# ICLDisco/ompi

Measured on AMD Instinct MI355X. Metric: Allreduce busBW GB/s @256MiB fp32 SUM at 2/4/8 GPUs; MPI_Op HBM GB/s, higher is better.
Workload: dtype f32; 1 GPU; MPI_Op 3-buffer SUM fp32, 1 GiB per buffer (BASELINE configs[1]); count=268435456, bytes_per_buffer=1073741824, op=MPI_SUM, datatype=MPI_FLOAT, kernel=op_vec_kernel<float,SUM,3buff>

## Files before the change

ompi_amd/csrc/coll_ipc.hip:

```cpp
#include <hip/hip_runtime.h>

#include <sched.h>
#include <unistd.h>

#include <algorithm>
#include <array>
#include <atomic>
#include <chrono>
#include <cstdarg>
#include <cstdio>
#include <cstdlib>
#include <cstring>
#include <deque>
#include <map>
#include <memory>
#include <mutex>
#include <new>
#include <utility>
#include <vector>

#include "../../include/ompi_amd_coll.h"
#include "bootstrap.h"
#include "comm_internal.h"
#include "host_mark.h"
// ... 1232 lines not shown
    if (want > kMaxIpcBytes) {
        record_msg("landing buffer of %zu bytes exceeds the %zu-byte IPC mapping limit", want,
                   kMaxIpcBytes);
        return OMPI_AMD_ERR_UNSUPPORTED;
    }
    land_blob mine{};
    char *fresh = nullptr;
    const hipError_t e = alloc_exportable(want, &fresh, &mine.d.h);
    mine.token = landing_token(c->rank);
    if (e == hipSuccess) land_desc(fresh, want, &mine.d);
    else record_hip(e, "landing buffer (deferred growth): hipMalloc / hipIpcGetMemHandle");
    mine.ok = e == hipSuccess;
    pending_op g{};
    g.kind = PEND_GROW;
    g.stream = s;
    g.grow = fresh;
    g.grow_bytes = want;
    g.grow_token = mine.token;
    const int rc = nb_ticket(c, g, &mine, sizeof(mine));
    if (rc != OMPI_AMD_SUCCESS) {
        release_exportable(fresh);
        return rc;
    }
    c->pending.push_back(g);
    c->npending.fetch_add(1);
    c->land_planned = want - kLandTag;
    return OMPI_AMD_SUCCESS;
}

static int launch_barrier(ompi_amd_comm_t *c, hipStream_t s);

static int grow_launch(ompi_amd_comm_t *c, const pending_op &g, const land_blob *all) {
    const size_t want = g.grow_bytes;
    ipc_ref *refs[kMaxRanks] = {};
    void *maps[kMaxRanks] = {};
    int status = all[c->rank].ok ? 0 : 1;
    for (int p = 0; p < c->size && status == 0; ++p) {
        if (p == c->rank) continue;
        if (!all[p].ok) {
            record_msg("landing buffer: rank %d failed to allocate or export its buffer", p);
            status = 1;
        } else if (ipc_map(alloc_of(all[p].d), c, &refs[p], &maps[p]) != OMPI_AMD_SUCCESS) {
            status = 1;
        }
    }
    if (status == 0) {
        tok_ptrs peers{};
        tok_set expect{};
        for (int p = 0; p < c->size; ++p) {
            expect.t[p] = all[p].token;
            if (p != c->rank) peers.p[p] = (const uint64_t *)((char *)maps[p] + want - kLandTag);
        }
        note_stream(c, g.stream);
        hipLaunchKernelGGL(land_stamp_kernel, dim3(1), dim3(1), 0, g.stream,
                           (uint64_t *)(g.grow + want - kLandTag), g.grow_token);
        int rc = record_hip(hipGetLastError(), "landing stamp launch (deferred growth)");
        if (rc == OMPI_AMD_SUCCESS) rc = launch_barrier(c, g.stream);
        if (rc == OMPI_AMD_SUCCESS) {
            hipLaunchKernelGGL(land_check_kernel, dim3(1), dim3(64), 0, g.stream, peers, expect, c->rank,
                               c->size, c->err_dev, c->flags + kAbortWord);
            rc = record_hip(hipGetLastError(), "landing check launch (deferred growth)");
        }
        if (rc != OMPI_AMD_SUCCESS) status = 1;
    }
    for (int q = 0; q < c->size; ++q) c->land_tokens.push_back(all[q].token);
    if (status != 0) {
        for (int p = 0; p < kMaxRanks; ++p) ipc_unmap(refs[p], c);
        if (g.grow) c->land_retired.push_back(g.grow);
        c->land_failed = true;
        return OMPI_AMD_ERR_HIP;
    }
    if (c->land) c->land_retired.push_back(c->land);
    for (int p = 0; p < kMaxRanks; ++p) {
        if (c->land_ref[p]) c->land_ref_retired.push_back(c->land_ref[p]);
        c->land_ref[p] = refs[p];
    }
    c->land = g.grow;
    for (int p = 0; p < c->size; ++p)
        c->peer_land.p[p] = p == c->rank ? c->land : (const char *)ipc_ref_base(c->land_ref[p]);
    c->land_bytes = want - kLandTag;
    ++c->deferred_growths;
    return OMPI_AMD_SUCCESS;
}

static int launch_barrier(ompi_amd_comm_t *c, hipStream_t s) {
    note_stream(c, s);
    ++c->epoch;
    const uint64_t ticks = (uint64_t)c->timeout_ms * 100000ull;
    hipLaunchKernelGGL(barrier_kernel, dim3(1), dim3(64), 0, s, c->flags, c->peer_flags, c->rank,
                       c->size, c->epoch, c->err_dev, ticks, c->dbg_dev);
    return record_hip(hipGetLastError(), "barrier launch");
}

static int launch_copy(ompi_amd_comm_t *c, const cp_jobs &jobs, hipStream_t s) {
    if (jobs.n == 0) return OMPI_AMD_SUCCESS;
    note_stream(c, s);
    int64_t most = 0;
    for (int i = 0; i < jobs.n; ++i) most = std::max(most, jobs.j[i].bytes);
    int64_t blocks = (most / 16 + kXferThreads * 4 - 1) / (kXferThreads * 4);
    blocks = std::max<int64_t>(1, std::min<int64_t>(blocks, std::max(1, c->max_blocks / jobs.n)));
    if (c->copy_nt)
        hipLaunchKernelGGL(copy_kernel<true>, dim3((unsigned)blocks, (unsigned)jobs.n),
                           dim3(kXferThreads), 0, s, jobs);
    else
        hipLaunchKernelGGL(copy_kernel<false>, dim3((unsigned)blocks, (unsigned)jobs.n),
                           dim3(kXferThreads), 0, s, jobs);
    return record_hip(hipGetLastError(), "copy launch");
}


static int arena_alloc(ompi_amd_comm_t *c, size_t need, char **out,
                       size_t min_chunk = (size_t)64 << 20) {
    host_step st("arena_alloc", need);
    const size_t n = (std::max<size_t>(need, 1) + 255) & ~(size_t)255;
    std::lock_guard<std::mutex> g(c->arena_mu);
    for (auto &ch : c->arena) {
        for (auto it = ch.free.begin(); it != ch.free.end(); ++it) {
            if (it->second < n) continue;
            const size_t off = it->first, left = it->second - n;
            ch.free.erase(it);
            if (left) ch.free[off + n] = left;
            ch.used[off] = n;
            *out = ch.base + off;
            return OMPI_AMD_SUCCESS;
        }
    }
    if (n > kMaxIpcBytes) {
        record_msg("shadow of %zu bytes exceeds the %zu-byte IPC allocation limit", n, kMaxIpcBytes);
        return OMPI_AMD_ERR_UNSUPPORTED;
    }
    const size_t want = std::min(kMaxIpcBytes,
                                 (std::max({n, min_chunk, c->arena_bytes}) + (2u << 20) - 1) &
                                     ~(size_t)((2u << 20) - 1));
    char *mem = nullptr;
    hipIpcMemHandle_t h;
    const hipError_t e = alloc_exportable(want, &mem, &h);
    if (e != hipSuccess) return record_hip(e, "shadow arena: hipMalloc / hipIpcGetMemHandle");
    c->arena.push_back({mem, want, {}, {}});
    auto &ch = c->arena.back();
    if (want > n) ch.free[n] = want - n;
    ch.used[0] = n;
    c->arena_bytes += want;
    *out = mem;
    return OMPI_AMD_SUCCESS;
}

static void arena_free(ompi_amd_comm_t *c, char *p) {
    if (!p) return;
    std::lock_guard<std::mutex> g(c->arena_mu);
    for (auto &ch : c->arena) {
        if (p < ch.base || p >= ch.base + ch.size) continue;
        const size_t off = (size_t)(p - ch.base);
        auto u = ch.used.find(off);
        if (u == ch.used.end()) return;
        size_t lo = off, len = u->second;
        ch.used.erase(u);
        auto nx = ch.free.lower_bound(off);
        if (nx != ch.free.end() && nx->first == off + len) {
            len += nx->second;
            nx = ch.free.erase(nx);
        }
        if (nx != ch.free.begin()) {
            auto pv = std::prev(nx);
            if (pv->first + pv->second == lo) {
                lo = pv->first;
                len += pv->second;
                ch.free.erase(pv);
            }
        }
        ch.free[lo] = len;
        return;
    }
}

static int shadow_reserve(ompi_amd_comm_t *c, size_t need, char **out, int k = 0) {
    char *&sh = k ? c->shadow2 : c->shadow;
    size_t &bytes = k ? c->shadow2_bytes : c->shadow_bytes;
    if (need <= bytes) {
        *out = sh;
        return OMPI_AMD_SUCCESS;
    }
    TRY(quiesce(c, "quiesce (shadow growth)"));
    arena_free(c, sh);
    const size_t want = std::max(need, std::min(2 * bytes, kMaxIpcBytes));
    sh = nullptr;
    bytes = 0;
    TRY(arena_alloc(c, want, &sh));
    bytes = want;
    *out = sh;
    return OMPI_AMD_SUCCESS;
}

static int shadow_plan(ompi_amd_comm_t *c, const void **src, size_t sbytes, void **rbuf,
                       size_t rbytes, bool rbuf_in, bool owned, shadow_set *post,
                       bool split_inplace = false) {
    *post = shadow_set{};
    bool inplace = *src && *src == (const void *)*rbuf;
    bool fs = false, fr = false;
    buf_desc d;
    if (*src && sbytes) {
        if (c->force_shadow || !c->user_ipc) {
            fs = true;
        } else {
            const int rc = export_buf(c, *src, &d, &fs);
            if (rc != OMPI_AMD_SUCCESS && !fs) return rc;
        }
    }
    if (inplace && fs && split_inplace) {
        inplace = false;
        fr = true;
        rbuf_in = false;
    } else if (inplace) {
        fr = fs;
        fs = false;
        rbytes = std::max(rbytes, sbytes);
        rbuf_in = true;
    } else if (*rbuf && rbytes) {
        if (c->force_shadow || !c->user_ipc) {
            fr = true;
        } else {
            const int rc = export_buf(c, *rbuf, &d, &fr);
            if (rc != OMPI_AMD_SUCCESS && !fr) return rc;
        }
    }
    if (!fs && !fr) return OMPI_AMD_SUCCESS;
    const size_t so = fs ? ((uintptr_t)*src & 255) : 0;
    const size_t rbase = fs ? ((so + sbytes + 255) & ~(size_t)255) : 0;
    const size_t ro = fr ? rbase + ((uintptr_t)*rbuf & 255) : rbase;
    size_t need = (fr ? ro + rbytes : so + sbytes) + 256;
    const bool split2 = fs && fr && need > kMaxIpcBytes;
    if (split2) need = so + sbytes + 256;
    char *mem = nullptr, *mem2 = nullptr;
    if (owned) {
        TRY(arena_alloc(c, need, &mem));
        post->mem = mem;
        if (split2) {
            TRY(arena_alloc(c, ((uintptr_t)*rbuf & 255) + rbytes + 256, &mem2));
            post->mem2 = mem2;
        }
    } else {
        TRY(shadow_reserve(c, need, &mem));
        if (split2) TRY(shadow_reserve(c, ((uintptr_t)*rbuf & 255) + rbytes + 256, &mem2, 1));
    }
    if (fs) {
        post->in.j[post->in.n++] = {(const char *)*src, mem + so, (int64_t)sbytes};
        *src = mem + so;
    }
    if (fr) {
        char *r = split2 ? mem2 + ((uintptr_t)*rbuf & 255) : mem + ro;
        if (rbuf_in) post->in.j[post->in.n++] = {(const char *)*rbuf, r, (int64_t)rbytes};
        post->out = {r, (char *)*rbuf, (int64_t)rbytes};
        *rbuf = r;
        if (inplace) *src = r;
    }
    ++c->shadowed;
    return OMPI_AMD_SUCCESS;
}

static int shadow_in(ompi_amd_comm_t *c, const shadow_set &sh, hipStream_t s) {
    return launch_copy(c, sh.in, s);
}

static int shadow_out(ompi_amd_comm_t *c, const shadow_set &sh, hipStream_t s) {
    if (sh.out.bytes <= 0) return OMPI_AMD_SUCCESS;
    cp_jobs cj{};
    cj.j[0] = sh.out;
    cj.n = 1;
    return launch_copy(c, cj, s);
}

static ptr_set one_ptr(const void *p) {
    ptr_set r{};
    r.p[0] = (const char *)p;
    return r;
}

static ptr_set push_order(const ompi_amd_comm_t *c, const ptr_set &bufs) {
    ptr_set r{};
    for (int k = 0; k < c->size; ++k) r.p[k] = bufs.p[(c->rank + k) % c->size];
    return r;
}

static int launch_reduce_core(int op, int type, const ptr_set &src, int nsrc, const ptr_set &dst,
                              int ndst, int order, int flags, red_jobs jobs, int max_blocks,
                              bool nt_store, hipStream_t s) {
    red_launch_fn f = red_fn(op, type);
    if (!f) return OMPI_AMD_ERR_UNSUPPORTED;
    if (jobs.n == 0 || nsrc < 1) return OMPI_AMD_SUCCESS;
    const size_t ext = ompi_amd_type_extent(type);
    int64_t most = 0;
    for (int i = 0; i < jobs.n; ++i) {
        red_job &j = jobs.j[i];
        const uintptr_t ph = (uintptr_t)(dst.p[0] + j.off_dst * ext) & 15;
        bool same = ext <= 16 && 16 % ext == 0;
        for (int r = 0; r < nsrc; ++r)
            same = same && ((((uintptr_t)(src.p[r] + j.off * ext)) & 15) == ph);
        for (int d = 1; d < ndst; ++d)
            same = same && ((((uintptr_t)(dst.p[d] + j.off_dst * ext)) & 15) == ph);
        const int64_t lead = (int64_t)((16 - ph) & 15);
        j.head = (same && lead % (int64_t)ext == 0) ? (int)std::min<int64_t>(lead / (int64_t)ext, j.cnt) : -1;
        most = std::max(most, j.cnt);
    }
    if (most == 0) return OMPI_AMD_SUCCESS;
    const int64_t per = (int64_t)(16 / ext) * kXferThreads;
    int64_t blocks = (most + per - 1) / per;
    blocks = std::max<int64_t>(1, std::min<int64_t>(blocks, std::max(1, max_blocks / jobs.n)));
    return record_hip(f(dim3((unsigned)blocks, (unsigned)jobs.n), src, dst, ndst, nsrc, order,
                        flags | (nt_store ? FOLD_NT_STORE : 0), jobs, s),
                      "reduce launch");
}

static int launch_reduce(ompi_amd_comm_t *c, int op, int type, const ptr_set &src, int nsrc,
                         const ptr_set &dst, int ndst, int order, int flags, const red_jobs &jobs,
                         hipStream_t s) {
    if (!red_fn(op, type)) return OMPI_AMD_ERR_UNSUPPORTED;
    if (jobs.n == 0 || nsrc < 1) return OMPI_AMD_SUCCESS;
    note_stream(c, s);
    return launch_reduce_core(op, type, src, nsrc, dst, ndst, order, flags, jobs, c->max_blocks,
                              c->copy_nt != 0, s);
}

static hipEvent_t prof_event(ompi_amd_comm_t *c) {
    if (!c->ev_free.empty()) {
        hipEvent_t e = c->ev_free.back();
        c->ev_free.pop_back();
        return e;
    }
    hipEvent_t e = nullptr;
    if (hipEventCreate(&e) != hipSuccess) return nullptr;
    return e;
}

template <typename F>
static int timed_phase(ompi_amd_comm_t *c, int phase, hipStream_t s, F &&launch) {
    if (!c->profile) return launch();
    hipEvent_t a = prof_event(c), b = prof_event(c);
    if (a) hip_ignore(hipEventRecord(a, s));
    const int rc = launch();
    if (b) hip_ignore(hipEventRecord(b, s));
    if (a && b) c->ev_phase[phase].emplace_back(a, b);
    return rc;
}

static int check_sticky(ompi_amd_comm_t *c) {
    const int e = __atomic_load_n(c->err_host, __ATOMIC_ACQUIRE);
    if (e != 0) {
        record_msg("collective device error %d (a peer did not reach a barrier within %lld ms)",
                   e, (long long)c->timeout_ms);
        return e;
    }
    return OMPI_AMD_SUCCESS;
}

static bool in_place(const void *sbuf, const void *rbuf) {
    return sbuf == rbuf || sbuf == (const void *)1;
}

struct stage_half {
    char *mine;
    ptr_set peers;
};
static stage_half next_half(ompi_amd_comm_t *c) {
    const size_t h = (size_t)(c->stage_seq++ & 1) * c->scratch_bytes;
    stage_half r;
    r.mine = c->scratch + h;
    for (int p = 0; p < kMaxRanks; ++p) r.peers.p[p] = c->peer_scratch.p[p] ? c->peer_scratch.p[p] + h : nullptr;
    return r;
}

static void ring_jobs(int64_t count, int n, red_jobs *jobs, int only_block) {
    int64_t split, early, late;
    blockcount(count, n, &split, &early, &late);
    jobs->n = 0;
    for (int b = 0; b < n; ++b) {
        if (only_block >= 0 && b != only_block) continue;
        red_job &j = jobs->j[jobs->n++];
        j.off = block_off(b, split, early, late);
        j.cnt = block_cnt(b, split, early, late);
        j.off_dst = j.off;
        j.first = b;
        j.head = -1;
    }
}

static int pof2_floor(int n) {
    int a = 1;
    while (a * 2 <= n) a *= 2;
    return a;
}

static fold_plan allreduce_fold(int n, int tuned_alg, size_t count, int type, bool root0_inplace,
                                int red_alg = 0) {
    const size_t msg = type_size(type) * count;
    const fold_plan tree{ORDER_TREE, 0, 0}, ring{ORDER_RING, 0, 0};
    const fold_plan linear{ORDER_CHAIN, 0, 0};
    switch (tuned_alg) {
    case TUNED_AR_BASIC_LINEAR: return linear;
    case TUNED_AR_NONOVERLAPPING: {
        const red_order ro = tuned_reduce_order(n, msg, count, 0, root0_inplace, red_alg);
        return {ro.order, ro.first, ro.flags};
    }
    case TUNED_AR_RECURSIVE_DOUBLING: return tree;
    case TUNED_AR_RING:
    case TUNED_AR_RING_SEGMENTED:
        return count < (size_t)n ? tree : ring;
    case TUNED_AR_RABENSEIFNER:
        return count < (size_t)pof2_floor(n) ? linear : fold_plan{ORDER_RABEN, 0, 0};
    default:
        return (msg < 10000 || count < (size_t)n) ? tree : ring;
    }
}

static void raben_piece(int64_t count, int n, int o, int64_t *lo, int64_t *cnt) {
    int64_t l = 0, w = count;
    for (int m = 1; m < pof2_floor(n); m <<= 1) {
        const int64_t half = w / 2;
        if (o & m) { l += half; w -= half; }
        else w = half;
    }
    *lo = l;
    *cnt = w;
}

static void fold_jobs(const fold_plan &p, int64_t count, int n, int block, red_jobs *jobs) {
    if (p.order == ORDER_RING) {
        ring_jobs(count, n, jobs, block);
        return;
    }
    int64_t lo = 0, hi = count;
    if (block >= 0) {
        int64_t split, early, late;
        blockcount(count, n, &split, &early, &late);
        lo = block_off(block, split, early, late);
        hi = lo + block_cnt(block, split, early, late);
    }
    jobs->n = 0;
    if (p.order != ORDER_RABEN) {
        red_job &j = jobs->j[jobs->n++];
        j = red_job{lo, hi - lo, lo, p.first, -1};
        return;
    }
    const int adj = pof2_floor(n);
    for (int o = 0; o < adj; ++o) {
        int64_t plo, pcnt;
        raben_piece(count, n, o, &plo, &pcnt);
        const int64_t a = std::max(lo, plo), b = std::min(hi, plo + pcnt);
        if (a >= b) continue;
        red_job &j = jobs->j[jobs->n++];
        j = red_job{a, b - a, a, 0, -1};
        j.aux = o << 8;
    }
}

static red_jobs one_job(int64_t off, int64_t cnt, int64_t off_dst, int first) {
    red_jobs jobs;
    jobs.n = 1;
    jobs.j[0] = {off, cnt, off_dst, first, -1};
    return jobs;
}
static int scan_sources(int rank, bool exclusive) { return exclusive ? rank : rank + 1; }

static int stage_in(ompi_amd_comm_t *c, const void *src, size_t bytes, stage_half *sh,
                    hipStream_t s) {
    if (bytes > c->scratch_bytes) {
        record_msg("staged collective of %zu B exceeds the %zu B scratch", bytes, c->scratch_bytes);
        return OMPI_AMD_ERR_BAD_PARAM;
    }
    *sh = next_half(c);
    cp_jobs cj{};
    cj.n = 1;
    cj.j[0] = {(const char *)src, sh->mine, (int64_t)bytes};
    TRY(launch_copy(c, cj, s));
    return launch_barrier(c, s);
}

static int allreduce_fused(ompi_amd_comm_t *c, const void *src, void *rbuf, int64_t count,
                           int op, int type, bool tree, hipStream_t s) {
    fused_launch_fn f = fused_fn(op, type);
    if (!f) return OMPI_AMD_ERR_UNSUPPORTED;
    note_stream(c, s);
    const int n = c->size;
    const stage_half sh = next_half(c);
    fused_args a{};
    a.src = (const char *)src;
    a.dst = (char *)rbuf;
    a.mine = sh.mine;
    a.peers = sh.peers;
    a.flags = c->flags;
    a.peer_flags = c->peer_flags;
    a.rank = c->rank;
    a.n = n;
    a.order = tree ? ORDER_TREE : ORDER_RING;
    a.count = count;
    blockcount(count, n, &a.split, &a.early, &a.late);
    a.epoch = ++c->epoch;
    a.timeout_ticks = (uint64_t)c->timeout_ms * 100000ull;
    a.err = c->err_dev;
    const int rows = tree ? 1 : n;
    const int64_t most = tree ? count : a.early;
    const int64_t cols = std::max<int64_t>(
        1, std::min<int64_t>((most + 4 * kXferThreads - 1) / (4 * kXferThreads),
                             kFusedMaxGroups / rows));
    if (c->want_mark && c->mark_word) {
        a.done = reinterpret_cast<uint32_t *>(c->flags) + kFusedDoneWord + kFusedDoneStride * c->mark_slot;
        a.mark = c->mark_word;
        a.mark_v = mark_reserve();
    }
    TRY(record_hip(f(dim3((unsigned)cols, (unsigned)rows), a, s), "fused allreduce launch"));
    if (a.mark) c->mark_embedded = a.mark_v;
    return OMPI_AMD_SUCCESS;
}

static size_t two_shot_result_off(size_t bytes) { return (bytes + 255) & ~(size_t)255; }

static bool two_shot_fits(const ompi_amd_comm_t *c, int64_t count, size_t ext) {
    int64_t split, early, late;
    blockcount(count, c->size, &split, &early, &late);
    return two_shot_result_off((size_t)count * ext) + (size_t)early * ext + 16 <= c->scratch_bytes;
}

static int allreduce_staged_two_shot(ompi_amd_comm_t *c, const void *src, void *rbuf,
                                     int64_t count, int op, int type, const fold_plan &fp,
                                     hipStream_t s) {
    const int n = c->size, mine = (c->rank + 1) % n;
    const int64_t ext = (int64_t)ompi_amd_type_extent(type);
    const size_t res = two_shot_result_off((size_t)count * ext);
    int64_t split, early, late;
    blockcount(count, n, &split, &early, &late);
    stage_half sh;
    TRY(stage_in(c, src, (size_t)(count * ext), &sh, s));
    const int64_t offm = block_off(mine, split, early, late) * ext;
    ptr_set dst{};
    dst.p[0] = (const char *)rbuf;
    dst.p[1] = sh.mine + res + (offm & 15) - offm;
    red_jobs jobs;
    fold_jobs(fp, count, n, mine, &jobs);
    TRY(launch_reduce(c, op, type, sh.peers, n, dst, 2, fp.order, fp.flags, jobs, s));
    TRY(launch_barrier(c, s));
    cp_jobs cj{};
    for (int b = 0; b < n; ++b) {
        if (b == mine) continue;
        const int owner = (b + n - 1) % n;
        const int64_t off = block_off(b, split, early, late) * ext;
        cj.j[cj.n++] = {sh.peers.p[owner] + res + (off & 15), (char *)rbuf + off,
                        block_cnt(b, split, early, late) * ext};
    }
    return launch_copy(c, cj, s);
}

static int allreduce_pull(ompi_amd_comm_t *c, const ptr_set &sp, const ptr_set &rp, void *rbuf,
                          int64_t count, int op, int type, const fold_plan &fp, hipStream_t s) {
    const int n = c->size, mine = (c->rank + 1) % n;
    const int64_t ext = (int64_t)ompi_amd_type_extent(type);
    TRY(launch_barrier(c, s));
    red_jobs jobs;
    fold_jobs(fp, count, n, mine, &jobs);
    TRY(timed_phase(c, 0, s, [&] {
        return launch_reduce(c, op, type, sp, n, one_ptr(rbuf), 1, fp.order, fp.flags, jobs, s);
    }));
    TRY(launch_barrier(c, s));
    int64_t split, early, late;
    blockcount(count, n, &split, &early, &late);
    cp_jobs cj{};
    for (int b = 0; b < n; ++b) {
        if (b == mine) continue;
        const int owner = (b + n - 1) % n;
        const int64_t off = block_off(b, split, early, late) * ext;
        cj.j[cj.n++] = {rp.p[owner] + off, (char *)rbuf + off, block_cnt(b, split, early, late) * ext};
    }
    TRY(timed_phase(c, 1, s, [&] { return launch_copy(c, cj, s); }));
    return launch_barrier(c, s);
}

static int allreduce_pull_staged(ompi_amd_comm_t *c, const ptr_set &sp, char *sh, void *rbuf,
                                 int64_t count, int op, int type, const fold_plan &fp,
                                 hipStream_t s) {
    const int n = c->size, mine = (c->rank + 1) % n;
    const int64_t ext = (int64_t)ompi_amd_type_extent(type);
    TRY(launch_barrier(c, s));
    red_jobs jobs;
    fold_jobs(fp, count, n, mine, &jobs);
    ptr_set dsts{};
    dsts.p[0] = (const char *)rbuf;
    dsts.p[1] = sh;
    TRY(timed_phase(c, 0, s, [&] {
        return launch_reduce(c, op, type, sp, n, dsts, 2, fp.order, fp.flags, jobs, s);
    }));
    TRY(launch_barrier(c, s));
    int64_t split, early, late;
    blockcount(count, n, &split, &early, &late);
    cp_jobs cj{};
    for (int b = 0; b < n; ++b) {
        if (b == mine) continue;
        const int owner = (b + n - 1) % n;
        const int64_t off = block_off(b, split, early, late) * ext;
        cj.j[cj.n++] = {sp.p[owner] + off, (char *)rbuf + off, block_cnt(b, split, early, late) * ext};
    }
    TRY(timed_phase(c, 1, s, [&] { return launch_copy(c, cj, s); }));
    return launch_barrier(c, s);
}

static int allreduce_pull_push(ompi_amd_comm_t *c, const ptr_set &sp, const ptr_set &rp,
                               int64_t count, int op, int type, const fold_plan &fp,
                               hipStream_t s) {
    const int n = c->size, mine = (c->rank + 1) % n;
    TRY(launch_barrier(c, s));
    red_jobs jobs;
    fold_jobs(fp, count, n, mine, &jobs);
    const ptr_set dsts = push_order(c, rp);
// ... 3026 lines not shown
```

ompi_amd/csrc/coll_kern.hip:

```cpp
#include <hip/hip_runtime.h>

#include <algorithm>
#include <array>
#include <utility>

#include "coll_kernels.h"

#ifndef COLL_OP
#error "build with -DCOLL_OP=<op index>"
#endif

namespace ompi_amd {
namespace {

template <int OP, int TYPE>
hipError_t red_launch_slot(dim3 grid, const ptr_set &src, const ptr_set &dst, int ndst, int n,
                           int order, int flags, const red_jobs &jobs, hipStream_t s) {
    if constexpr (slot_supported(OP, TYPE)) {
        using T = typename type_of<TYPE>::type;
        if (n <= 8)
            hipLaunchKernelGGL((reduce_kernel<T, OP, 8>), grid, dim3(kXferThreads), 0, s, src, dst,
                               ndst, n, order, flags, jobs);
        else
            hipLaunchKernelGGL((reduce_kernel<T, OP, kMaxRanks>), grid, dim3(kXferThreads), 0, s,
                               src, dst, ndst, n, order, flags, jobs);
        return hipGetLastError();
    } else {
        return hipErrorInvalidValue;
    }
}

template <int OP, int TYPE>
hipError_t fused_launch_slot(dim3 grid, const fused_args &a, hipStream_t s) {
    if constexpr (slot_supported(OP, TYPE)) {
        using T = typename type_of<TYPE>::type;
        hipLaunchKernelGGL((fused_allreduce_kernel<T, OP>), grid, dim3(kXferThreads), 0, s, a);
        return hipGetLastError();
    } else {
        return hipErrorInvalidValue;
    }
}

template <int OP, int TYPE>
hipError_t pipe_launch_slot(unsigned groups, const pipe_args &a, hipStream_t s) {
    if constexpr (slot_supported(OP, TYPE)) {
        using T = typename type_of<TYPE>::type;
        if (a.n > 8) return hipErrorInvalidValue;
        static const int64_t cap = [] {
            int per_cu = 0, cus = 0, dev = 0;
            if (hipGetDevice(&dev) != hipSuccess ||
                hipOccupancyMaxActiveBlocksPerMultiprocessor(
                    &per_cu, reinterpret_cast<const void *>(&pipe_allreduce_kernel<T, OP, 8>),
                    kXferThreads, 0) != hipSuccess ||
                hipDeviceGetAttribute(&cus, hipDeviceAttributeMultiprocessorCount, dev) != hipSuccess) {
                (void)hipGetLastError();
                return (int64_t)64;
            }
            return std::max<int64_t>(1, (int64_t)per_cu * cus / 2);
        }();
        const int64_t fit = std::max<int64_t>(1, cap / std::max(1, a.colocated));
        const dim3 g((unsigned)std::min<int64_t>(groups, fit)), b(kXferThreads);
        hipLaunchKernelGGL((pipe_allreduce_kernel<T, OP, 8>), g, b, 0, s, a);
        return hipGetLastError();
    } else {
        return hipErrorInvalidValue;
    }
}

template <int OP, int... T>
constexpr std::array<red_launch_fn, OMPI_AMD_TYPE_COUNT> make_red_row(std::integer_sequence<int, T...>) {
    return {{(slot_supported(OP, T) ? &red_launch_slot<OP, T> : (red_launch_fn) nullptr)...}};
}
template <int OP, int... T>
constexpr std::array<fused_launch_fn, OMPI_AMD_TYPE_COUNT> make_fused_row(
    std::integer_sequence<int, T...>) {
    return {{(slot_supported(OP, T) ? &fused_launch_slot<OP, T> : (fused_launch_fn) nullptr)...}};
}

template <int OP, int... T>
constexpr std::array<pipe_launch_fn, OMPI_AMD_TYPE_COUNT> make_pipe_row(
    std::integer_sequence<int, T...>) {
    return {{(slot_supported(OP, T) ? &pipe_launch_slot<OP, T> : (pipe_launch_fn) nullptr)...}};
}

const auto g_red_row = make_red_row<COLL_OP>(std::make_integer_sequence<int, OMPI_AMD_TYPE_COUNT>{});
const auto g_fused_row = make_fused_row<COLL_OP>(std::make_integer_sequence<int, OMPI_AMD_TYPE_COUNT>{});
const auto g_pipe_row = make_pipe_row<COLL_OP>(std::make_integer_sequence<int, OMPI_AMD_TYPE_COUNT>{});

}

#define ROW_NAME2(a, b) a##b
#define ROW_NAME(a, b) ROW_NAME2(a, b)
const red_launch_fn *ROW_NAME(red_row_, COLL_OP)() { return g_red_row.data(); }
const fused_launch_fn *ROW_NAME(fused_row_, COLL_OP)() { return g_fused_row.data(); }
const pipe_launch_fn *ROW_NAME(pipe_row_, COLL_OP)() { return g_pipe_row.data(); }

}
```

ompi_amd/csrc/coll_kernels.h:

```cpp
#pragma once

#include <hip/hip_runtime.h>

#include <cstdint>

#include "../../include/ompi_amd_coll.h"
#include "op_device.h"

namespace ompi_amd {

constexpr int kMaxRanks = OMPI_AMD_MAX_RANKS;
constexpr int kXferThreads = 256;

struct ptr_set { const char *p[kMaxRanks]; };
struct flag_set { uint64_t *p[kMaxRanks]; };

enum order_t {
    ORDER_RING = 0,
    ORDER_TREE = 1,
    ORDER_CHAIN = 2,
    ORDER_BINOMIAL = 3,
    ORDER_BINARY = 4,
    ORDER_HALVING = 5,
    ORDER_RABEN = 6,
};
constexpr int FOLD_ROOT_INPLACE = 1;
constexpr int FOLD_NT_STORE = 1 << 16;

struct red_job {
    int64_t off, cnt, off_dst;
    int first;
    int head;
    int aux = 0;
};
struct red_jobs { red_job j[2 * kMaxRanks]; int n; };

struct cp_job { const char *src; char *dst; int64_t bytes; };
struct cp_jobs { cp_job j[kMaxRanks]; int n; };

__device__ __forceinline__ void sys_acquire() {
    __builtin_amdgcn_fence(__ATOMIC_ACQUIRE, "");
    asm volatile("s_waitcnt vmcnt(0)" ::: "memory");
}
__device__ __forceinline__ void sys_release() {
    __builtin_amdgcn_fence(__ATOMIC_RELEASE, "");
    asm volatile("s_waitcnt vmcnt(0)" ::: "memory");
}

__device__ __forceinline__ void acquire_once() {
    if (threadIdx.x == 0) sys_acquire();
    __syncthreads();
}

constexpr int kAbortWord = 512;
constexpr size_t kFlagPageBytes = 8192;

__device__ __forceinline__ bool wait_epoch(const uint64_t *flag, uint64_t epoch, int *err,
                                           uint64_t ticks, uint64_t *abort_word,
                                           uint64_t *seen = nullptr) {
    const uint64_t t0 = __builtin_amdgcn_s_memrealtime();
    uint64_t check = t0 + 100000;
    while (__hip_atomic_load(flag, __ATOMIC_RELAXED, __HIP_MEMORY_SCOPE_SYSTEM) < epoch) {
        __builtin_amdgcn_s_sleep(1);
        const uint64_t now = __builtin_amdgcn_s_memrealtime();
        if (now - t0 > ticks) {
            __hip_atomic_store(err, (int)OMPI_AMD_ERR_TIMEOUT, __ATOMIC_RELAXED,
                               __HIP_MEMORY_SCOPE_SYSTEM);
            __hip_atomic_store(abort_word, (uint64_t)1, __ATOMIC_RELAXED, __HIP_MEMORY_SCOPE_SYSTEM);
            return false;
        }
        if (now >= check) {
            if (seen)
                __hip_atomic_store(seen, __hip_atomic_load(flag, __ATOMIC_RELAXED, __HIP_MEMORY_SCOPE_SYSTEM),
                                   __ATOMIC_RELAXED, __HIP_MEMORY_SCOPE_SYSTEM);
            if (__hip_atomic_load(abort_word, __ATOMIC_RELAXED, __HIP_MEMORY_SCOPE_SYSTEM) != 0) {
                __hip_atomic_store(err, (int)OMPI_AMD_ERR_TIMEOUT, __ATOMIC_RELAXED,
                                   __HIP_MEMORY_SCOPE_SYSTEM);
                return false;
            }
            check = now + 100000;
        }
    }
    return true;
}

__device__ __forceinline__ void xfer_epilogue() {
    asm volatile("s_waitcnt vmcnt(0)" ::: "memory");
    __syncthreads();
    if (threadIdx.x == 0) sys_release();
}

template <typename T, int OP, int NM = kMaxRanks>
__device__ __forceinline__ T fold(const T (&v)[NM], int n, int order, int flags) {
    using F = opfn<OP, false>;
    const bool swap = (flags & FOLD_ROOT_INPLACE) != 0;
    if (order == ORDER_RING) {
        T acc = v[0];
#pragma unroll
        for (int j = 1; j < NM; ++j)
            if (j < n) acc = F::template f<T>(v[j], acc);
        return acc;
    }
    if (order == ORDER_CHAIN) {
        T acc = v[NM - 1];
#pragma unroll
        for (int j = NM - 1; j >= 0; --j) {
            if (j == n - 1) acc = v[j];
            else if (j < n - 1) acc = (j == 0 && swap) ? F::template f<T>(v[0], acc)
                                                       : F::template f<T>(acc, v[j]);
        }
        return acc;
    }
    if (order == ORDER_BINOMIAL) {
        T w[NM];
#pragma unroll
        for (int i = 0; i < NM; ++i) w[i] = v[i];
#pragma unroll
        for (int u = 0; u + 1 < NM; u += 2)
            if (u + 1 < n) w[u] = (u == 0 && swap) ? F::template f<T>(w[0], w[1])
                                                   : F::template f<T>(w[u + 1], w[u]);
#pragma unroll
        for (int m = 2; m < NM; m <<= 1) {
#pragma unroll
            for (int u = 0; u + m < NM; u += 2 * m)
                if (u + m < n) w[u] = F::template f<T>(w[u], w[u + m]);
        }
        return w[0];
    }
    if (order == ORDER_BINARY) {
        T w[NM];
#pragma unroll
        for (int i = 0; i < NM; ++i) w[i] = v[i];
#pragma unroll
        for (int s = NM - 1; s >= 0; --s) {
            int d = 1;
            while (2 * d <= s + 1) d *= 2;
            const int c0 = s + d, c1 = s + 2 * d;
            if (c0 < NM && c0 < n)
                w[s] = (s == 0 && swap) ? F::template f<T>(w[0], w[c0])
                                        : F::template f<T>(w[c0], w[s]);
            if (c1 < NM && c1 < n) w[s] = F::template f<T>(w[s], w[c1]);
        }
        return w[0];
    }
    if (order == ORDER_RABEN) {
        int adj = 1;
        while (adj * 2 <= n) adj *= 2;
        const int rem = n - adj;
        const int o = (flags >> 8) & 0xff;
        const bool right = (o & 1) != 0;
        T w[NM];
#pragma unroll
        for (int u = 0; u < NM; ++u) {
            if (2 * u + 1 < NM && u < rem)
                w[u] = right ? F::template f<T>(v[2 * u + 1], v[2 * u])
                             : F::template f<T>(v[2 * u], v[2 * u + 1]);
            else if (u < adj)
                w[u] = v[u + rem < NM ? u + rem : 0];
        }
#pragma unroll
        for (int m = 1; m < NM; m <<= 1) {
            if (m < adj) {
#pragma unroll
                for (int u = 0; u < NM; ++u)
                    if (u < adj && (u & m) == (o & m)) w[u] = F::template f<T>(w[u], w[u ^ m]);
            }
        }
        T r = w[0];
#pragma unroll
        for (int u = 1; u < NM; ++u)
            if (u == o) r = w[u];
        return r;
    }
    if (order == ORDER_HALVING) {
        int adj = 1;
        while (adj * 2 <= n) adj *= 2;
        const int remain = n - adj;
        const int tb = (flags >> 8) & 0xff;
        T w[NM];
#pragma unroll
        for (int u = 0; u < NM; ++u) {
            if (2 * u + 1 < NM && u < remain) w[u] = F::template f<T>(v[2 * u + 1], v[2 * u]);
            else if (u < adj) w[u] = v[u + remain];
        }
#pragma unroll
        for (int m = NM / 2; m >= 1; m >>= 1) {
            if (m < adj) {
#pragma unroll
                for (int u = 0; u < NM; ++u)
                    if (u < adj && (u & m) == (tb & m)) w[u] = F::template f<T>(w[u], w[u ^ m]);
            }
        }
        T r = w[0];
#pragma unroll
        for (int u = 1; u < NM; ++u)
            if (u == tb) r = w[u];
        return r;
    }
    int adj = 1;
    while (adj * 2 <= n) adj *= 2;
    const int extra = n - adj;
    T w[NM];
#pragma unroll
    for (int i = 0; i < NM; ++i) {
        if (i < extra) w[i] = F::template f<T>(v[2 * i + 1], v[2 * i]);
        else if (i < adj) w[i] = v[i + extra];
    }
#pragma unroll
    for (int len = NM; len > 1; len >>= 1) {
        if (len <= adj) {
#pragma unroll
            for (int i = 0; i < NM / 2; ++i)
                if (2 * i + 1 < len) w[i] = F::template f<T>(w[2 * i + 1], w[2 * i]);
        }
    }
    return w[0];
}

template <typename T, int NM = kMaxRanks>
__device__ __forceinline__ void gather_scalar(T (&v)[NM], const ptr_set &src, int n,
                                              int first, int64_t e) {
#pragma unroll
    for (int j = 0; j < NM; ++j) {
        if (j < n) {
            const int r = (first + j) % n;
            v[j] = reinterpret_cast<const T *>(src.p[r])[e];
        }
    }
}

template <typename T, int OP, int NM = kMaxRanks>
__global__ __launch_bounds__(kXferThreads) void reduce_kernel(ptr_set src, ptr_set dst, int ndst,
                                                              int n, int order, int flags,
                                                              red_jobs jobs) {
    acquire_once();
    const red_job jb = jobs.j[blockIdx.y];
    constexpr int E = 16 / sizeof(T);
    const int64_t gstride = (int64_t)gridDim.x * kXferThreads;
    const int64_t tid = (int64_t)blockIdx.x * kXferThreads + threadIdx.x;
    const int64_t head = jb.head < 0 ? jb.cnt : jb.head;
    const int64_t nvec = jb.head < 0 ? 0 : (jb.cnt - head) / E;
    for (int64_t i = tid; i < nvec; i += gstride) {
        vec16<T> v[NM];
#pragma unroll
        for (int j = 0; j < NM; ++j) {
            if (j < n) {
                const int r = (jb.first + j) % n;
                const u32x4 *p = reinterpret_cast<const u32x4 *>(
                    reinterpret_cast<const T *>(src.p[r]) + jb.off + head);
                v[j].v = __builtin_nontemporal_load(p + i);
            }
        }
        vec16<T> out;
#pragma unroll
        for (int e = 0; e < E; ++e) {
            T s[NM];
#pragma unroll
            for (int j = 0; j < NM; ++j) s[j] = v[j].e[e];
            out.e[e] = fold<T, OP, NM>(s, n, order, flags | jb.aux);
        }
        if (flags & FOLD_NT_STORE) {
#pragma unroll
            for (int k = 0; k < NM; ++k)
                if (k < ndst)
                    __builtin_nontemporal_store(
                        out.v, reinterpret_cast<u32x4 *>(reinterpret_cast<T *>(const_cast<char *>(dst.p[k])) +
                                                         jb.off_dst + head) + i);
        } else {
#pragma unroll
            for (int k = 0; k < NM; ++k)
                if (k < ndst)
                    reinterpret_cast<u32x4 *>(reinterpret_cast<T *>(const_cast<char *>(dst.p[k])) +
                                              jb.off_dst + head)[i] = out.v;
        }
    }
    const int64_t tail0 = head + nvec * E;
    const int64_t nscalar = head + (jb.cnt - tail0);
    for (int64_t k = tid; k < nscalar; k += gstride) {
        const int64_t e = k < head ? k : tail0 + (k - head);
        T s[NM];
        gather_scalar<T, NM>(s, src, n, jb.first, jb.off + e);
        const T r = fold<T, OP, NM>(s, n, order, flags | jb.aux);
#pragma unroll
        for (int d = 0; d < NM; ++d)
            if (d < ndst)
                store_elem<T>(reinterpret_cast<T *>(const_cast<char *>(dst.p[d])) + jb.off_dst + e,
                              r);
    }
    xfer_epilogue();
}

constexpr int kFusedMaxGroups = 4096 / (int)sizeof(uint64_t) / kMaxRanks;

struct fused_args {
    const char *src;
    char *dst, *mine;
    ptr_set peers;
    uint64_t *flags;
    flag_set peer_flags;
    int rank, n, order;
    int64_t count, split, early, late;
    uint64_t epoch, timeout_ticks;
    int *err;
    uint32_t *done;
    uint64_t *mark;
    uint64_t mark_v;
};

constexpr int kFusedDoneWord = 8192 / (int)sizeof(uint32_t);
constexpr int kFusedDoneStride = 64 / (int)sizeof(uint32_t);
constexpr int kFusedDoneSlots = (64 << 10) / 64 - 8192 / 64;

template <typename T, int OP>
__global__ __launch_bounds__(kXferThreads) void fused_allreduce_kernel(fused_args a) {
    const int t = threadIdx.x;
    const int g = blockIdx.y * gridDim.x + blockIdx.x;
    int64_t off = 0, cnt = a.count;
    int first = 0;
    if (a.order == ORDER_RING) {
        const int64_t b = blockIdx.y;
        off = b < a.split ? b * a.early : b * a.late + a.split;
        cnt = b < a.split ? a.early : a.late;
        first = (int)b;
    }
    const int64_t per = (cnt + gridDim.x - 1) / gridDim.x;
    const int64_t lo = off + min(cnt, per * (int64_t)blockIdx.x);
    const int64_t hi = off + min(cnt, per * (int64_t)(blockIdx.x + 1));
    const T *src = reinterpret_cast<const T *>(a.src);
    T *mine = reinterpret_cast<T *>(a.mine);
    for (int64_t e = lo + t; e < hi; e += kXferThreads) mine[e] = src[e];
    asm volatile("s_waitcnt vmcnt(0)" ::: "memory");
    __syncthreads();
    if (t == 0) sys_release();
    __syncthreads();
    __shared__ int gave_up;
    if (t == 0) gave_up = 0;
    __syncthreads();
    if (t < a.n && t != a.rank) {
        __hip_atomic_store(a.peer_flags.p[t] + g * kMaxRanks + a.rank, a.epoch, __ATOMIC_RELAXED,
                           __HIP_MEMORY_SCOPE_SYSTEM);
        if (!wait_epoch(a.flags + g * kMaxRanks + t, a.epoch, a.err, a.timeout_ticks,
                        a.flags + kAbortWord))
            gave_up = 1;
    }
    __syncthreads();
    if (gave_up) return;
    acquire_once();
    T *dst = reinterpret_cast<T *>(a.dst);
    for (int64_t e = lo + t; e < hi; e += kXferThreads) {
        T v[kMaxRanks];
        gather_scalar<T>(v, a.peers, a.n, first, e);
        store_elem<T>(dst + e, fold<T, OP>(v, a.n, a.order, 0));
    }
    if (a.mark) {
        asm volatile("s_waitcnt vmcnt(0)" ::: "memory");
        __syncthreads();
        if (t == 0) {
            __builtin_amdgcn_fence(__ATOMIC_RELEASE, "agent");
            const uint32_t total = gridDim.x * gridDim.y;
            if (__hip_atomic_fetch_add(a.done, 1u, __ATOMIC_ACQ_REL, __HIP_MEMORY_SCOPE_AGENT) == total - 1) {
                __hip_atomic_store(a.done, 0u, __ATOMIC_RELAXED, __HIP_MEMORY_SCOPE_AGENT);
                __hip_atomic_store(a.mark, a.mark_v, __ATOMIC_RELAXED, __HIP_MEMORY_SCOPE_SYSTEM);
            }
        }
    }
}

constexpr int kPipeMaxGroups = 1024;
constexpr size_t kPipeFlagOff = 64 << 10;
constexpr size_t kPipeFlagBytes = 2 * (size_t)kPipeMaxGroups * kMaxRanks * sizeof(uint64_t);

struct pipe_args {
    const char *src;
    ptr_set dst_c;
    ptr_set src_f;
    ptr_set dst_f;
    ptr_set src_g;
    char *rbuf;
    uint64_t *flags;
    flag_set peer_flags;
    int rank, n, mine, ndst, order, first, fold_flags, nt;
    int colocated;
    int64_t split, early, late;
    int64_t per, nslices;
    uint64_t seq, timeout_ticks;
    int *err;
    uint64_t *abort_word;
};

__device__ __forceinline__ size_t pipe_row(int phase, int w, int r) {
    return ((size_t)phase * kPipeMaxGroups + (size_t)w) * kMaxRanks + (size_t)r;
}

__device__ __forceinline__ void pipe_copy(const char *s, char *d, int64_t lo, int64_t hi, bool nt) {
    const int t = threadIdx.x;
    if (hi <= lo) return;
    int64_t head = hi - lo, nv = 0;
    if ((((uintptr_t)(s + lo) ^ (uintptr_t)(d + lo)) & 15) == 0) {
        head = min(hi - lo, (int64_t)((16 - ((uintptr_t)(s + lo) & 15)) & 15));
        nv = (hi - lo - head) / 16;
    }
    const u32x4 *sv = reinterpret_cast<const u32x4 *>(s + lo + head);
    u32x4 *dv = reinterpret_cast<u32x4 *>(d + lo + head);
    constexpr int S = kXferThreads;
    int64_t i = t;
    for (; i + 3 * S < nv; i += 4 * S) {
        const u32x4 a = __builtin_nontemporal_load(sv + i);
        const u32x4 b = __builtin_nontemporal_load(sv + i + S);
        const u32x4 c = __builtin_nontemporal_load(sv + i + 2 * S);
        const u32x4 e = __builtin_nontemporal_load(sv + i + 3 * S);
        if (nt) {
            __builtin_nontemporal_store(a, dv + i);
            __builtin_nontemporal_store(b, dv + i + S);
            __builtin_nontemporal_store(c, dv + i + 2 * S);
            __builtin_nontemporal_store(e, dv + i + 3 * S);
        } else {
            dv[i] = a;
            dv[i + S] = b;
            dv[i + 2 * S] = c;
            dv[i + 3 * S] = e;
        }
    }
    for (; i < nv; i += S) {
        if (nt) __builtin_nontemporal_store(__builtin_nontemporal_load(sv + i), dv + i);
        else dv[i] = __builtin_nontemporal_load(sv + i);
    }
    const int64_t tail0 = lo + head + nv * 16;
    const int64_t nrest = head + (hi - tail0);
    for (int64_t k = t; k < nrest; k += S) {
        const int64_t b = k < head ? lo + k : tail0 + (k - head);
        d[b] = s[b];
    }
}

template <typename T, int OP, int NM>
__device__ __forceinline__ void pipe_fold(const pipe_args &a, int64_t lo, int64_t hi) {
    constexpr int E = 16 / sizeof(T);
    const int t = threadIdx.x;
    if (hi <= lo) return;
    const uintptr_t ph = (uintptr_t)(a.dst_f.p[0] + lo * (int64_t)sizeof(T)) & 15;
    bool same = true;
#pragma unroll
    for (int j = 0; j < NM; ++j)
        if (j < a.n) same = same && (((uintptr_t)(a.src_f.p[j] + lo * (int64_t)sizeof(T)) & 15) == ph);
#pragma unroll
    for (int k = 1; k < NM; ++k)
        if (k < a.ndst) same = same && (((uintptr_t)(a.dst_f.p[k] + lo * (int64_t)sizeof(T)) & 15) == ph);
    const int64_t lead = (int64_t)((16 - ph) & 15);
    int64_t head = hi - lo, nv = 0;
    if (same && lead % (int64_t)sizeof(T) == 0) {
        head = min(hi - lo, lead / (int64_t)sizeof(T));
        nv = (hi - lo - head) / E;
    }
    const int64_t v0 = lo + head;
    for (int64_t i = t; i < nv; i += kXferThreads) {
        vec16<T> v[NM];
#pragma unroll
        for (int j = 0; j < NM; ++j) {
            if (j < a.n) {
                const int r = (a.first + j) % a.n;
                const u32x4 *p = reinterpret_cast<const u32x4 *>(reinterpret_cast<const T *>(a.src_f.p[r]) + v0);
                v[j].v = __builtin_nontemporal_load(p + i);
            }
        }
        vec16<T> out;
#pragma unroll
        for (int e = 0; e < E; ++e) {
            T s[NM];
#pragma unroll
            for (int j = 0; j < NM; ++j) s[j] = v[j].e[e];
            out.e[e] = fold<T, OP, NM>(s, a.n, a.order, a.fold_flags);
        }
#pragma unroll
        for (int k = 0; k < NM; ++k) {
            if (k < a.ndst) {
                u32x4 *q = reinterpret_cast<u32x4 *>(reinterpret_cast<T *>(const_cast<char *>(a.dst_f.p[k])) + v0) + i;
                if (a.nt) __builtin_nontemporal_store(out.v, q);
                else *q = out.v;
            }
        }
    }
    const int64_t tail0 = v0 + nv * E;
    const int64_t nrest = head + (hi - tail0);
    for (int64_t k = t; k < nrest; k += kXferThreads) {
        const int64_t e = k < head ? lo + k : tail0 + (k - head);
        T s[NM];
        gather_scalar<T, NM>(s, a.src_f, a.n, a.first, e);
        const T r = fold<T, OP, NM>(s, a.n, a.order, a.fold_flags);
#pragma unroll
        for (int d = 0; d < NM; ++d)
            if (d < a.ndst) store_elem<T>(reinterpret_cast<T *>(const_cast<char *>(a.dst_f.p[d])) + e, r);
    }
}

template <typename T, int OP, int NM>
__global__ __launch_bounds__(kXferThreads) void pipe_allreduce_kernel(pipe_args a) {
    const int t = threadIdx.x, w = blockIdx.x, G = gridDim.x;
    const int64_t P = (a.nslices - w + G - 1) / G;
    constexpr int64_t ext = sizeof(T);
    __shared__ int gave_up;
    if (t == 0) gave_up = 0;
    __syncthreads();
    for (int64_t p = 0; p < P + 2; ++p) {
        const bool doC = p < P, doF = p >= 1 && p <= P, doG = p >= 2;
        if (p >= 1) {
            if (t < a.n && t != a.rank) {
                bool ok = true;
                if (doF)
                    ok = wait_epoch(a.flags + pipe_row(0, w, t), a.seq + (uint64_t)p, a.err,
                                    a.timeout_ticks, a.abort_word);
                if (ok && doG)
                    ok = wait_epoch(a.flags + pipe_row(1, w, t), a.seq + (uint64_t)(p - 1), a.err,
                                    a.timeout_ticks, a.abort_word);
                if (!ok) gave_up = 1;
            }
            __syncthreads();
            if (gave_up) return;
            acquire_once();
        }
        if (doC) {
            const int64_t s = w + p * G;
#pragma unroll
            for (int b = 0; b < NM; ++b) {
                if (b >= a.n || !a.dst_c.p[b]) continue;
                const int64_t off = b < a.split ? b * a.early : b * a.late + a.split;
                const int64_t cnt = b < a.split ? a.early : a.late;
                const int64_t lo = off + min(cnt, s * a.per), hi = off + min(cnt, (s + 1) * a.per);
                pipe_copy(a.src, const_cast<char *>(a.dst_c.p[b]), lo * ext, hi * ext, a.nt);
            }
        }
        if (doF) {
            const int64_t s = w + (p - 1) * G;
            const int b = a.mine;
            const int64_t off = b < a.split ? b * a.early : b * a.late + a.split;
            const int64_t cnt = b < a.split ? a.early : a.late;
            pipe_fold<T, OP, NM>(a, off + min(cnt, s * a.per), off + min(cnt, (s + 1) * a.per));
        }
        if (doG) {
            const int64_t s = w + (p - 2) * G;
#pragma unroll
            for (int b = 0; b < NM; ++b) {
                if (b >= a.n || !a.src_g.p[b]) continue;
                const int64_t off = b < a.split ? b * a.early : b * a.late + a.split;
                const int64_t cnt = b < a.split ? a.early : a.late;
                const int64_t lo = off + min(cnt, s * a.per), hi = off + min(cnt, (s + 1) * a.per);
                pipe_copy(a.src_g.p[b], a.rbuf, lo * ext, hi * ext, a.nt);
            }
        }
        if (doC || doF) {
            asm volatile("s_waitcnt vmcnt(0)" ::: "memory");
            __syncthreads();
            if (t == 0) sys_release();
            __syncthreads();
            if (t < a.n && t != a.rank) {
                if (doC)
                    __hip_atomic_store(a.peer_flags.p[t] + pipe_row(0, w, a.rank), a.seq + (uint64_t)(p + 1),
                                       __ATOMIC_RELAXED, __HIP_MEMORY_SCOPE_SYSTEM);
                if (doF)
                    __hip_atomic_store(a.peer_flags.p[t] + pipe_row(1, w, a.rank), a.seq + (uint64_t)p,
                                       __ATOMIC_RELAXED, __HIP_MEMORY_SCOPE_SYSTEM);
            }
        }
    }
    xfer_epilogue();
}

struct a2a_args {
    const char *sbuf;
    char *rbuf, *mine;
    ptr_set peers;
    uint64_t *flags;
    flag_set peer_flags;
    int rank, n;
    int self_copy;
    int64_t slot;
    int64_t scount[kMaxRanks], sdispl[kMaxRanks], rcount[kMaxRanks], rdispl[kMaxRanks];
// ... 186 lines not shown
```

Before: 6398 GB/s.

## Unroll reduce kernel loads and specialize rank count by source count

The reduce kernel now processes U chunks per thread, issuing all nontemporal loads for every chunk before an explicit vmcnt wait and the folds, which raises memory-level parallelism. Rank-count template instantiations (2/4/8/16) are chosen from nsrc, so small reductions use fewer registers and a larger unroll, and pointers are hoisted into the global address space. The grid-size calculation moves into a shared header and accounts for the unroll, so fewer blocks are launched. This adds more template instantiations and higher register pressure per thread, and the clamped duplicate loads in the tail chunk do redundant work.

```diff
diff --git a/ompi_amd/csrc/coll_fold_grid.h b/ompi_amd/csrc/coll_fold_grid.h
--- /dev/null
+++ b/ompi_amd/csrc/coll_fold_grid.h
@@ -0,0 +1,20 @@
+#pragma once
+#include <algorithm>
+#include <cstdint>
+
+namespace ompi_amd {
+
+constexpr int kFoldThreads = 256;
+
+constexpr int fold_nm(int n, int64_t ext) {
+    return n > 8 ? 16 : ext > 8 ? 8 : n <= 2 ? 2 : n <= 4 ? 4 : 8;
+}
+constexpr int fold_unroll(int nm) { return nm <= 8 ? 8 / nm : 1; }
+
+inline int64_t fold_grid_blocks(int64_t most, int64_t ext, int nsrc, int max_blocks, int njobs) {
+    const int64_t per = std::max<int64_t>(1, 16 / ext) * kFoldThreads * fold_unroll(fold_nm(nsrc, ext));
+    const int64_t blocks = (most + per - 1) / per;
+    return std::max<int64_t>(1, std::min<int64_t>(blocks, std::max(1, max_blocks / njobs)));
+}
+
+}
diff --git a/ompi_amd/csrc/coll_ipc.hip b/ompi_amd/csrc/coll_ipc.hip
--- a/ompi_amd/csrc/coll_ipc.hip
+++ b/ompi_amd/csrc/coll_ipc.hip
@@ -1558,9 +1558,7 @@
         most = std::max(most, j.cnt);
     }
     if (most == 0) return OMPI_AMD_SUCCESS;
-    const int64_t per = (int64_t)(16 / ext) * kXferThreads;
-    int64_t blocks = (most + per - 1) / per;
-    blocks = std::max<int64_t>(1, std::min<int64_t>(blocks, std::max(1, max_blocks / jobs.n)));
+    const int64_t blocks = fold_grid_blocks(most, (int64_t)ext, nsrc, max_blocks, jobs.n);
     return record_hip(f(dim3((unsigned)blocks, (unsigned)jobs.n), src, dst, ndst, nsrc, order,
                         flags | (nt_store ? FOLD_NT_STORE : 0), jobs, s),
                       "reduce launch");
diff --git a/ompi_amd/csrc/coll_kern.hip b/ompi_amd/csrc/coll_kern.hip
--- a/ompi_amd/csrc/coll_kern.hip
+++ b/ompi_amd/csrc/coll_kern.hip
@@ -18,12 +18,16 @@
                            int order, int flags, const red_jobs &jobs, hipStream_t s) {
     if constexpr (slot_supported(OP, TYPE)) {
         using T = typename type_of<TYPE>::type;
-        if (n <= 8)
-            hipLaunchKernelGGL((reduce_kernel<T, OP, 8>), grid, dim3(kXferThreads), 0, s, src, dst,
-                               ndst, n, order, flags, jobs);
-        else
-            hipLaunchKernelGGL((reduce_kernel<T, OP, kMaxRanks>), grid, dim3(kXferThreads), 0, s,
-                               src, dst, ndst, n, order, flags, jobs);
+#define RED_LAUNCH(NM)                                                                            \
+    hipLaunchKernelGGL((reduce_kernel<T, OP, NM, fold_unroll(NM)>), grid, dim3(kXferThreads), 0, \
+                       s, src, dst, ndst, n, order, flags, jobs)
+        switch (fold_nm(n, (int64_t)sizeof(T))) {
+        case 2: if constexpr (sizeof(T) <= 8) RED_LAUNCH(2); break;
+        case 4: if constexpr (sizeof(T) <= 8) RED_LAUNCH(4); break;
+        case 8: RED_LAUNCH(8); break;
+        default: RED_LAUNCH(kMaxRanks); break;
+        }
+#undef RED_LAUNCH
         return hipGetLastError();
     } else {
         return hipErrorInvalidValue;
diff --git a/ompi_amd/csrc/coll_kernels.h b/ompi_amd/csrc/coll_kernels.h
--- a/ompi_amd/csrc/coll_kernels.h
+++ b/ompi_amd/csrc/coll_kernels.h
@@ -5,12 +5,14 @@
 #include <cstdint>
 
 #include "../../include/ompi_amd_coll.h"
+#include "coll_fold_grid.h"
 #include "op_device.h"
 
 namespace ompi_amd {
 
 constexpr int kMaxRanks = OMPI_AMD_MAX_RANKS;
 constexpr int kXferThreads = 256;
+static_assert(kFoldThreads == kXferThreads && fold_nm(kMaxRanks, 4) == kMaxRanks, "coll_fold_grid.h");
 
 struct ptr_set { const char *p[kMaxRanks]; };
 struct flag_set { uint64_t *p[kMaxRanks]; };
@@ -229,7 +231,7 @@
     }
 }
 
-template <typename T, int OP, int NM = kMaxRanks>
+template <typename T, int OP, int NM = kMaxRanks, int U = 1>
 __global__ __launch_bounds__(kXferThreads) void reduce_kernel(ptr_set src, ptr_set dst, int ndst,
                                                               int n, int order, int flags,
                                                               red_jobs jobs) {
@@ -240,38 +242,50 @@
     const int64_t tid = (int64_t)blockIdx.x * kXferThreads + threadIdx.x;
     const int64_t head = jb.head < 0 ? jb.cnt : jb.head;
     const int64_t nvec = jb.head < 0 ? 0 : (jb.cnt - head) / E;
-    for (int64_t i = tid; i < nvec; i += gstride) {
-        vec16<T> v[NM];
-#pragma unroll
-        for (int j = 0; j < NM; ++j) {
-            if (j < n) {
-                const int r = (jb.first + j) % n;
-                const u32x4 *p = reinterpret_cast<const u32x4 *>(
-                    reinterpret_cast<const T *>(src.p[r]) + jb.off + head);
-                v[j].v = __builtin_nontemporal_load(p + i);
-            }
-        }
-        vec16<T> out;
-#pragma unroll
-        for (int e = 0; e < E; ++e) {
-            T s[NM];
-#pragma unroll
-            for (int j = 0; j < NM; ++j) s[j] = v[j].e[e];
-            out.e[e] = fold<T, OP, NM>(s, n, order, flags | jb.aux);
-        }
-        if (flags & FOLD_NT_STORE) {
-#pragma unroll
-            for (int k = 0; k < NM; ++k)
-                if (k < ndst)
-                    __builtin_nontemporal_store(
-                        out.v, reinterpret_cast<u32x4 *>(reinterpret_cast<T *>(const_cast<char *>(dst.p[k])) +
-                                                         jb.off_dst + head) + i);
-        } else {
-#pragma unroll
-            for (int k = 0; k < NM; ++k)
-                if (k < ndst)
-                    reinterpret_cast<u32x4 *>(reinterpret_cast<T *>(const_cast<char *>(dst.p[k])) +
-                                              jb.off_dst + head)[i] = out.v;
+    using gvec = __attribute__((address_space(1))) u32x4;
+    const gvec *sv[NM];
+    gvec *dv[NM];
+#pragma unroll
+    for (int j = 0; j < NM; ++j) {
+        if (j < n)
+            sv[j] = (const gvec *)(reinterpret_cast<const T *>(src.p[(jb.first + j) % n]) + jb.off + head);
+        if (j < ndst)
+            dv[j] = (gvec *)(reinterpret_cast<T *>(const_cast<char *>(dst.p[j])) + jb.off_dst + head);
+    }
+    constexpr int64_t chunk = (int64_t)kXferThreads * U;
+    const int64_t cstride = (int64_t)gridDim.x * chunk;
+    for (int64_t i0 = (int64_t)blockIdx.x * chunk + threadIdx.x; i0 < nvec; i0 += cstride) {
+        vec16<T> v[U][NM];
+#pragma unroll
+        for (int u = 0; u < U; ++u) {
+            const int64_t i = min(i0 + (int64_t)u * kXferThreads, nvec - 1);
+#pragma unroll
+            for (int j = 0; j < NM; ++j)
+                if (j < n) v[u][j].v = __builtin_nontemporal_load(sv[j] + i);
+        }
+        __builtin_amdgcn_s_waitcnt(0x0F70);
+#pragma unroll
+        for (int u = 0; u < U; ++u) {
+            const int64_t i = i0 + (int64_t)u * kXferThreads;
+            vec16<T> out;
+#pragma unroll
+            for (int e = 0; e < E; ++e) {
+                T s[NM];
+#pragma unroll
+                for (int j = 0; j < NM; ++j) s[j] = v[u][j].e[e];
+                out.e[e] = fold<T, OP, NM>(s, n, order, flags | jb.aux);
+            }
+            if (i < nvec) {
+                if (flags & FOLD_NT_STORE) {
+#pragma unroll
+                    for (int k = 0; k < NM; ++k)
+                        if (k < ndst) __builtin_nontemporal_store(out.v, dv[k] + i);
+                } else {
+#pragma unroll
+                    for (int k = 0; k < NM; ++k)
+                        if (k < ndst) dv[k][i] = out.v;
+                }
+            }
         }
     }
     const int64_t tail0 = head + nvec * E;
```

New measurement: 6453 GB/s, median of 2. Within noise of the previous version (+0.9%).
